# USharma002/CUDA-PathTracer

Measured on AMD Instinct MI355X. Metric: Msamples/s, higher is better.
Workload: dtype f32

## Files before the change

### cuda-pathtracer_amd/csrc/bounce.h

```cpp
#pragma once
#include "shading.h"

namespace ptmi {

struct BounceArgs {
    DeviceScene sc; TileMap tm; PathState st; FrameParams fp;
    const int* queue_in; int n_in;
    const int* count_in;
    int* queue_out; int* count_out;
    int segments;
    StatCounters* stats;
    int many_waves;
    int* done_count;
    int* next_count;
    int* host_count;
    int* cursor;
    unsigned int* cost; unsigned int* cost_max;
};

using BounceKernel = void (*)(BounceArgs);
#pragma GCC visibility push(hidden)
BounceKernel select_bounce_sync(const BounceArgs& a);
BounceKernel select_bounce_phased(const BounceArgs& a);
BounceKernel select_bounce_wide(const BounceArgs& a);
#pragma GCC visibility pop

inline bool is_guided(const BounceArgs& a) { return a.fp.sampling_mode != 0 && a.sc.cdfs != nullptr; }

#ifdef PTMI_TRACE_WAVES
#define PTMI_TR(...) __VA_ARGS__
#else
#define PTMI_TR(...)
#endif

template <bool LDS_GEOM>
__device__ __forceinline__ float4* stage_scene(const DeviceScene& sc, float4* lds, const float4*& nodes, const float4*& prims, const float4*& mats) {
    nodes = sc.nodes; prims = sc.prims; mats = sc.mats;
    if (LDS_GEOM) {
        const int n_node_vec = 2 * sc.n_nodes, n_prim_vec = sc.prim_stride * sc.n_prims, n_mat_vec = 3 * sc.n_prims;
        for (int i = threadIdx.x; i < n_node_vec; i += kBlock) lds[i] = sc.nodes[i];
        for (int i = threadIdx.x; i < n_prim_vec; i += kBlock) lds[n_node_vec + i] = sc.prims[i];
        for (int i = threadIdx.x; i < n_mat_vec; i += kBlock) lds[n_node_vec + n_prim_vec + i] = sc.mats[i];
        nodes = lds; prims = lds + n_node_vec; mats = lds + n_node_vec + n_prim_vec;
        lds += n_node_vec + n_prim_vec + n_mat_vec;
        __syncthreads();
    }
    return lds;
}

template <bool STATS, bool COMPACT = true>
__device__ __forceinline__ void finish_launch(const BounceArgs& a, bool alive, int slot, const LaneCounters& cn) {
    if (COMPACT) {
        const unsigned long long mask = __ballot(alive);
        const int lane = threadIdx.x & 63;
        int base = 0;
        if (lane == 0 && mask) base = atomicAdd(a.count_out, __popcll(mask));
        base = __shfl(base, 0);
        if (alive) a.queue_out[base + __popcll(mask & ((1ull << lane) - 1ull))] = slot;
    }
    if (STATS) {
        unsigned long long r = cn.rays, nv = cn.node_visits, pt = cn.prim_tests, h = cn.hits, tv = cn.top_visits;
        unsigned long long cc = cn.cert_chain, cf = cn.cert_fallback;
        for (int off = 32; off > 0; off >>= 1) {
            r += __shfl_down(r, off); nv += __shfl_down(nv, off); pt += __shfl_down(pt, off); h += __shfl_down(h, off); tv += __shfl_down(tv, off);
            cc += __shfl_down(cc, off); cf += __shfl_down(cf, off);
        }
        if ((threadIdx.x & 63) == 0) {
            atomicAdd(&a.stats->rays, r); atomicAdd(&a.stats->node_visits, nv);
            atomicAdd(&a.stats->prim_tests, pt); atomicAdd(&a.stats->hits, h);
            if (tv) atomicAdd(&a.stats->top_node_visits, tv);
            if (cc) atomicAdd(&a.stats->cert_chain, cc);
            if (cf) atomicAdd(&a.stats->cert_fallback, cf);
        }
    }
}

__device__ __forceinline__ void publish_count(const BounceArgs& a) {
    if (!a.host_count) return;
    if ((threadIdx.x & 63) == 0) {
        __threadfence();
        if (atomicAdd(a.done_count, 1) == (int)(gridDim.x * (kBlock / 64)) - 1) {
            const int c = atomicAdd(a.count_out, 0);
            atomicExch(a.next_count, 0); atomicExch(a.next_count + 1, 0);
            atomicExch(a.done_count, 0);
            __hip_atomic_store(a.host_count, c, __ATOMIC_RELEASE, __HIP_MEMORY_SCOPE_SYSTEM);
        }
    }
}

__device__ __forceinline__ bool end_visit(const BounceArgs& a, int n_in, bool more, int& slot, PathRegs& p, int& segs_left) {
    store_path(a.st, slot, p);
    if (a.cost) {
        const unsigned int c = a.cost[slot] + (unsigned int)(a.segments - segs_left);
        a.cost[slot] = c;
        if (!more) atomicMax(a.cost_max, c);
    }
    const int lane = threadIdx.x & 63;
    const unsigned long long ending = __ballot(1), surviving = __ballot(more);
    const int first = __ffsll((long long)ending) - 1;
    int out_base = 0, in_base = 0;
    if (lane == first) {
        if (surviving) out_base = atomicAdd(a.count_out, __popcll(surviving));
        if (a.cursor) in_base = atomicAdd(a.cursor, __popcll(ending));
    }
    out_base = __shfl(out_base, first); in_base = __shfl(in_base, first);
    if (more) a.queue_out[out_base + __popcll(surviving & ((1ull << lane) - 1ull))] = slot;
    const int entry = (int)(gridDim.x * kBlock) + in_base + __popcll(ending & ((1ull << lane) - 1ull));
    if (!(a.cursor && entry < n_in)) return false;
    slot = a.queue_in ? a.queue_in[entry] : entry;
    load_path(a.st, a.tm, slot, p);
    segs_left = a.segments;
    return true;
}

}
```

### cuda-pathtracer_amd/csrc/bounce_sync.hip

```cpp
#include "bounce.h"

namespace ptmi {

template <int MODE, bool LDS_GEOM, bool HAS_QUADS, bool STATS, bool GUIDED, bool BATCH>
__device__ __forceinline__ void bounce_body(const BounceArgs& a) {
    extern __shared__ float4 smem[];
    static_assert(MODE != TRAVERSAL_SWEEP || LDS_GEOM, "the sweep reads the scene through LDS broadcasts");
    const int n_in = a.count_in ? *a.count_in : a.n_in;
    if ((int)(blockIdx.x * kBlock) >= n_in) return;
    const int idx = blockIdx.x * kBlock + threadIdx.x;
    const bool active = idx < n_in;
    const float4 *nodes, *prims, *mats;
    float4* lds = stage_scene<LDS_GEOM>(a.sc, smem, nodes, prims, mats);
    int* stack = reinterpret_cast<int*>(lds) + threadIdx.x;
    if (GUIDED) fill_grid_solid_angles();

    const int slot = active ? (a.queue_in ? a.queue_in[idx] : idx) : 0;
    bool alive = active;
    PathRegs p = {};
    if (active) load_path(a.st, a.tm, slot, p);
    LaneCounters cn = {0, 0, 0, 0, 0, 0, 0};

    for (int seg = 0; seg < a.segments; seg++) {
        if (!__any(alive)) break;
        float t = 0.0f; int k = -1;
        if (STATS && alive) cn.rays++;
        const bool hit = scene_intersect<MODE, HAS_QUADS, STATS>(nodes, prims, a.sc.prim_stride, a.sc.n_nodes, stack, alive,
                                                               p.o, p.d, 1e-4f, FLT_MAX, t, k, cn);
        constexpr bool LEAN = MODE == TRAVERSAL_SWEEP && !STATS && !GUIDED;
        if (alive) alive = shade_step<STATS, GUIDED, false, BATCH, LEAN>(a.fp, a.tm, MatSource{mats, nullptr, nullptr}, a.sc.cdfs, p, hit, t, k, cn, slot);
    }

    if (active) store_path(a.st, slot, p);
    finish_launch<STATS>(a, alive, slot, cn);
}
template <int MODE, bool LDS_GEOM, bool HAS_QUADS, bool STATS, bool GUIDED, bool BATCH>
__global__ __launch_bounds__(kBlock, GUIDED ? 6 : (BATCH && MODE == TRAVERSAL_SWEEP ? 8 : 1)) __attribute__((amdgpu_num_sgpr(80))) void ptmi_bounce(BounceArgs a) {
    bounce_body<MODE, LDS_GEOM, HAS_QUADS, STATS, GUIDED, BATCH>(a);
    publish_count(a);
}

BounceKernel select_bounce_sync(const BounceArgs& a) {
    const auto pick = [&](auto mode, auto geom) {
        return with_bool(a.sc.has_quads, [&](auto quads) {
            return with_bool(a.stats != nullptr, [&](auto stats) {
                return with_bool(is_guided(a), [&](auto guided) {
                    return with_bool(a.fp.n_frames > 1, [&](auto batch) -> BounceKernel {
                        return ptmi_bounce<decltype(mode)::value, decltype(geom)::value, decltype(quads)::value, decltype(stats)::value,
                                           decltype(guided)::value, decltype(batch)::value>;
                    });
                });
            });
        });
    };
    switch (a.sc.traversal) {
        case TRAVERSAL_SWEEP: return pick(std::integral_constant<int, TRAVERSAL_SWEEP>{}, std::true_type{});
        case TRAVERSAL_LANE: return with_bool(a.sc.lds_resident, [&](auto geom) { return pick(std::integral_constant<int, TRAVERSAL_LANE>{}, geom); });
        default: return with_bool(a.sc.lds_resident, [&](auto geom) { return pick(std::integral_constant<int, TRAVERSAL_STACK>{}, geom); });
    }
}

}
```

### cuda-pathtracer_amd/csrc/debug_hooks.hip

```cpp
#include "light_sample.h"
#include "../../include/ptmi.h"

namespace ptmi {

template <int MODE, bool HAS_QUADS>
__global__ __launch_bounds__(kBlock) void ptmi_debug_intersect_k(DeviceScene sc, int n, const float* o, const float* d, float t_min,
                                                                 float t_max, int* hit, int* prim, float* t_out, float* p_out, float* n_out) {
    extern __shared__ float4 smem[];
    int* stack = reinterpret_cast<int*>(smem) + threadIdx.x;
    const int i = blockIdx.x * kBlock + threadIdx.x;
    const bool live = i < n;
    const int j = live ? i : 0;
    const f3 ro = mk3(o[3 * j], o[3 * j + 1], o[3 * j + 2]), rd = mk3(d[3 * j], d[3 * j + 1], d[3 * j + 2]);
    LaneCounters cn = {0, 0, 0, 0, 0, 0, 0};
    float t = 0.0f; int k = -1;
    const bool h = scene_intersect<MODE, HAS_QUADS, false>(sc.nodes, sc.prims, sc.prim_stride, sc.n_nodes, stack, live, ro, rd, t_min, t_max, t, k, cn);
    if (!live) return;
    hit[i] = h ? 1 : 0;
    prim[i] = h ? __float_as_int(sc.mats[3 * k].w) : -1;
    t_out[i] = h ? t : 0.0f;
    const f3 p = h ? ro + t * rd : mk3(0, 0, 0);
    const f3 nn = h ? xyz(sc.mats[3 * k]) : mk3(0, 0, 0);
    p_out[3 * i] = p.x; p_out[3 * i + 1] = p.y; p_out[3 * i + 2] = p.z;
    n_out[3 * i] = nn.x; n_out[3 * i + 1] = nn.y; n_out[3 * i + 2] = nn.z;
}

void launch_debug_intersect(const DeviceScene& sc, int n, const float* o, const float* d, float t_min, float t_max,
                            int* hit, int* prim, float* t, float* p, float* nrm, hipStream_t s) {
    if (n <= 0) return;
    const size_t lds = (size_t)sc.stack_entries * kBlock * sizeof(int);
    const dim3 grid((n + kBlock - 1) / kBlock), block(kBlock);
    const int walk = sc.traversal == TRAVERSAL_PHASED || sc.traversal == TRAVERSAL_PACKED || sc.traversal == TRAVERSAL_CERTIFIED ? TRAVERSAL_LANE : sc.traversal;
    const auto launch = [&](auto mode) {
        with_bool(sc.has_quads, [&](auto quads) {
            hipLaunchKernelGGL((ptmi_debug_intersect_k<decltype(mode)::value, decltype(quads)::value>), grid, block, lds, s, sc, n, o, d, t_min, t_max, hit, prim, t, p, nrm);
        });
    };
    if (walk == TRAVERSAL_SWEEP) launch(std::integral_constant<int, TRAVERSAL_SWEEP>{});
    else if (walk == TRAVERSAL_LANE) launch(std::integral_constant<int, TRAVERSAL_LANE>{});
    else launch(std::integral_constant<int, TRAVERSAL_STACK>{});
}

template <bool QUADS>
__global__ __launch_bounds__(kBlock) void ptmi_debug_intersect_wide_k(DeviceScene sc, int n, const float* o, const float* d, float t_min,
                                                                      float t_max, int* hit, int* prim, float* t_out,
                                                                      unsigned long long* counts ) {
    extern __shared__ float4 smem[];
    const int i = blockIdx.x * kBlock + threadIdx.x;
    if (i >= n) return;
    const f3 ro = mk3(o[3 * i], o[3 * i + 1], o[3 * i + 2]), rd = mk3(d[3 * i], d[3 * i + 1], d[3 * i + 2]);
    float closest_t = t_max;
    bool tie = false;
    WideCounts wc = {0, 0};
    const int slot_hit = wide_closest_hit<QUADS, true>(sc, reinterpret_cast<uint2*>(smem) + threadIdx.x, ro, rd, t_min, closest_t, tie, wc);
    hit[i] = slot_hit >= 0 ? 1 : 0;
    prim[i] = slot_hit >= 0 ? sc.wload_index[slot_hit] : -1;
    t_out[i] = slot_hit >= 0 ? closest_t : 0.0f;
    if (counts) { atomicAdd(&counts[0], (unsigned long long)wc.node_visits); atomicAdd(&counts[1], (unsigned long long)wc.prim_tests); }
}
void launch_debug_intersect_wide(const DeviceScene& sc, int n, const float* o, const float* d, float t_min, float t_max,
                                 int* hit, int* prim, float* t, unsigned long long* counts, hipStream_t s) {
    if (n <= 0) return;
    const size_t lds = (size_t)sc.w_depth * kBlock * sizeof(uint2);
    const dim3 grid((n + kBlock - 1) / kBlock), block(kBlock);
    with_bool(sc.has_quads, [&](auto quads) {
        hipLaunchKernelGGL(ptmi_debug_intersect_wide_k<decltype(quads)::value>, grid, block, lds, s, sc, n, o, d, t_min, t_max, hit, prim, t, counts);
    });
}

__global__ void ptmi_debug_rng_k(const uint32_t* __restrict__ jump, unsigned long long seed_base, int n_pixels,
                                 const int* pixels, int count, float* out) {
    const int i = blockIdx.x * blockDim.x + threadIdx.x;
    if (i >= n_pixels) return;
    const unsigned int pix = (unsigned int)pixels[i];
    const unsigned long long seed = seed_base + (unsigned long long)pix;
    const uint32_t s0 = ((uint32_t)seed) ^ 0xaad26b49u, s1 = (uint32_t)(seed >> 32) ^ 0xf7dcefddu;
    const uint32_t t0 = 1099087573u * s0, t1 = 2591861531u * s1;
    uint32_t v[5] = {123456789u + t0, 362436069u ^ t0, 521288629u + t1, 88675123u ^ t1, 5783321u + t0};
    for (int k = 0; k < 32; k++) {
        if (!((pix >> k) & 1u)) continue;
        uint32_t r[5] = {0, 0, 0, 0, 0};
        for (int w = 0; w < 5; w++)
            for (int b = 0; b < 32; b++)
                if ((v[w] >> b) & 1u) for (int c = 0; c < 5; c++) r[c] ^= jump[(k * 160 + w * 32 + b) * 5 + c];
        for (int w = 0; w < 5; w++) v[w] = r[w];
    }
    Rng rng = {v[0], v[1], v[2], v[3], v[4], 6615241u + t1 + t0};
    for (int c = 0; c < count; c++) out[(size_t)i * count + c] = rng_uniform(rng);
}

void launch_debug_rng(const uint32_t* d_jump, uint64_t seed_base, int n_pixels, const int* pixels, int count, float* out, hipStream_t s) {
    if (n_pixels <= 0) return;
    hipLaunchKernelGGL(ptmi_debug_rng_k, dim3((n_pixels + 63) / 64), dim3(64), 0, s, d_jump, (unsigned long long)seed_base,
                       n_pixels, pixels, count, out);
}

__global__ void ptmi_debug_rcp_k(unsigned int first, unsigned long long count, unsigned long long* out ) {
    const unsigned long long stride = (unsigned long long)gridDim.x * blockDim.x;
    unsigned long long bad = 0, first_bad = ~0ull;
    for (unsigned long long i = blockIdx.x * (unsigned long long)blockDim.x + threadIdx.x; i < count; i += stride) {
        const unsigned int bits = first + (unsigned int)i;
        const float a = __uint_as_float(bits);
        const float want = 1.0f / a, got = rcp_exact_normal(a);
        if (__float_as_uint(want) != __float_as_uint(got) && !(want != want && got != got)) { bad++; if (first_bad == ~0ull) first_bad = bits; }
    }
    if (bad) { atomicAdd(&out[0], bad); atomicMin(&out[1], first_bad); }
}
void launch_debug_rcp(unsigned int first, unsigned long long count, unsigned long long* d_out, hipStream_t s) {
    hipLaunchKernelGGL(ptmi_debug_rcp_k, dim3(4096), dim3(256), 0, s, first, count, d_out);
}

__global__ void ptmi_debug_sqrt_k(unsigned int first, unsigned long long count, unsigned long long* out ) {
    const unsigned long long stride = (unsigned long long)gridDim.x * blockDim.x;
    unsigned long long bad = 0, first_bad = ~0ull;
    for (unsigned long long i = blockIdx.x * (unsigned long long)blockDim.x + threadIdx.x; i < count; i += stride) {
// ... 271 lines not shown
```

### cuda-pathtracer_amd/csrc/kernels.hip

```cpp
#include "bounce.h"

namespace ptmi {

__global__ __launch_bounds__(kBlock) void ptmi_render_init(TileMap tm, PathState st, const uint32_t* __restrict__ jump,
                                                           unsigned long long seed_base) {
    __shared__ uint32_t M[160 * 5];
    const int n = tm.local_rows * tm.width;
    const int slot = blockIdx.x * kBlock + threadIdx.x;
    const bool live = slot < n;
    int x = 0, y = 0;
    const unsigned int pix = live ? (unsigned int)global_pixel(tm, slot, x, y) : 0u;
    const unsigned long long seed = seed_base + (unsigned long long)pix;
    const uint32_t s0 = ((uint32_t)seed) ^ 0xaad26b49u;
    const uint32_t s1 = (uint32_t)(seed >> 32) ^ 0xf7dcefddu;
    const uint32_t t0 = 1099087573u * s0;
    const uint32_t t1 = 2591861531u * s1;
    uint32_t v[5] = {123456789u + t0, 362436069u ^ t0, 521288629u + t1, 88675123u ^ t1, 5783321u + t0};
    const uint32_t d = 6615241u + t1 + t0;

    for (int k = 0; k < 32; k++) {
        const bool mine = live && ((pix >> k) & 1u);
        if (!__syncthreads_or(mine ? 1 : 0)) continue;
        for (int i = threadIdx.x; i < 160 * 5; i += kBlock) M[i] = jump[k * 160 * 5 + i];
        __syncthreads();
        if (mine) {
            uint32_t r[5] = {0u, 0u, 0u, 0u, 0u};
#pragma unroll
            for (int w = 0; w < 5; w++) {
                const uint32_t word = v[w];
                for (int b = 0; b < 32; b++) {
                    const uint32_t m = 0u - ((word >> b) & 1u);
                    const uint32_t* row = &M[(w * 32 + b) * 5];
                    r[0] ^= row[0] & m; r[1] ^= row[1] & m; r[2] ^= row[2] & m; r[3] ^= row[3] & m; r[4] ^= row[4] & m;
                }
            }
#pragma unroll
            for (int w = 0; w < 5; w++) v[w] = r[w];
        }
        __syncthreads();
    }
    if (!live) return;
    st.E[slot] = make_uint4(v[0], v[1], v[2], v[3]);
    st.F[slot] = make_uint2(v[4], d);
    st.A[slot] = make_float4(0, 0, 0, 1.0f);
    st.B[slot] = make_float4(0, 0, 1.0f, 1.0f);
    st.C[slot] = make_float4(0, 0, 0, 1.0f);
    st.D[slot] = make_float4(0, 0, 0, __uint_as_float(0u));
}

__global__ __launch_bounds__(kBlock) void ptmi_frame_begin(TileMap tm, PathState st, FrameParams fp) {
    const int n = tm.local_rows * tm.width;
    const int slot = blockIdx.x * kBlock + threadIdx.x;
    if (slot >= n) return;
    int x, y;
    global_pixel(tm, slot, x, y);
    const uint4 e = st.E[slot]; const uint2 f = st.F[slot];
    Rng rng = {e.x, e.y, e.z, e.w, f.x, f.y};
    f3 o, d;
    camera_ray(fp, tm, x, y, rng, o, d);
    st.A[slot] = make_float4(o.x, o.y, o.z, 1.0f);
    st.B[slot] = make_float4(d.x, d.y, d.z, 1.0f);
    st.C[slot] = make_float4(0.0f, 0.0f, 0.0f, 1.0f);
    st.D[slot] = make_float4(0.0f, 0.0f, 0.0f, __uint_as_float(0u));
    st.E[slot] = make_uint4(rng.v0, rng.v1, rng.v2, rng.v3);
    st.F[slot] = make_uint2(rng.v4, rng.d);
}

size_t bounce_lds_bytes_wide(const DeviceScene& sc) { return (size_t)sc.w_top * kWideNodeDwords * 4 + (size_t)sc.w_depth * kBlock * sizeof(uint2); }
size_t bounce_lds_bytes(const DeviceScene& sc) {
    if (sc.traversal == TRAVERSAL_WIDE || sc.traversal == TRAVERSAL_CERTIFIED) return bounce_lds_bytes_wide(sc);
    size_t b = 0;
    const bool geom = sc.lds_resident || sc.traversal == TRAVERSAL_SWEEP;
    if (geom) b += (size_t)(2 * sc.n_nodes + (sc.prim_stride + 3) * sc.n_prims) * sizeof(float4);
    if (sc.traversal == TRAVERSAL_STACK) b += (size_t)sc.stack_entries * kBlock * sizeof(int);
    return b;
}

static BounceKernel select_bounce_kernel(const BounceArgs& a, size_t* lds) {
    const DeviceScene& sc = a.sc;
    *lds = bounce_lds_bytes(sc);
    switch (sc.traversal) {
        case TRAVERSAL_PHASED: return select_bounce_phased(a);
        case TRAVERSAL_PACKED: *lds = (size_t)sc.n_top * 2 * sizeof(float4); return select_bounce_phased(a);
        case TRAVERSAL_WIDE:
        case TRAVERSAL_CERTIFIED: return select_bounce_wide(a);
        default: return select_bounce_sync(a);
    }
}

void launch_bounce(const DeviceScene& sc, const TileMap& tm, const PathState& st, const FrameParams& fp,
                   const int* queue_in, int n_in, const int* count_in, int* queue_out, int* count_out, int segments,
                   StatCounters* stats, bool many_waves, hipStream_t s, const CountPublish& pub, const LaunchSchedule& sched) {
    if (n_in <= 0) return;
    BounceArgs a{sc, tm, st, fp, queue_in, n_in, count_in, queue_out, count_out, segments, stats, many_waves ? 1 : 0,
                 pub.done_count, pub.next_count, pub.host_count, nullptr, nullptr, nullptr};
    dim3 grid((n_in + kBlock - 1) / kBlock);
    const bool wide = sc.traversal == TRAVERSAL_WIDE || sc.traversal == TRAVERSAL_CERTIFIED;
    if (wide && sched.max_waves > 0 && sched.cursor) {
        a.cursor = sched.cursor;
        grid.x = std::min<unsigned int>(grid.x, (unsigned int)(sched.max_waves + kBlock / 64 - 1) / (kBlock / 64));
    }
    if (wide) { a.cost = sched.cost; a.cost_max = sched.cost_max; }
    size_t lds = 0;
    const BounceKernel k = select_bounce_kernel(a, &lds);
    hipLaunchKernelGGL(k, grid, dim3(kBlock), lds, s, a);
}

int bounce_resident_waves(const DeviceScene& sc, const FrameParams& fp, bool stats, int n_cus) {
    BounceArgs a{sc, TileMap(), PathState(), fp, nullptr, 0, nullptr, nullptr, nullptr, 0, stats ? reinterpret_cast<StatCounters*>(1) : nullptr, 0,
                 nullptr, nullptr, nullptr, nullptr, nullptr, nullptr};
    size_t lds = 0;
    const BounceKernel k = select_bounce_kernel(a, &lds);
    int blocks = 0;
    if (hipOccupancyMaxActiveBlocksPerMultiprocessor(&blocks, k, kBlock, lds) != hipSuccess) blocks = 0;
    return blocks * (kBlock / 64) * n_cus;
}

__device__ __forceinline__ int cost_class(unsigned int c, unsigned int cmax, int shift) {
    const unsigned long long k = ((unsigned long long)min(c, cmax) << 8) / ((unsigned long long)cmax + 1ull);
    return (255 - (int)k) >> shift;
}
__global__ __launch_bounds__(kBlock) void ptmi_cost_histogram(const int* __restrict__ queue_in, int n, const unsigned int* __restrict__ cost,
                                                              const unsigned int* __restrict__ cost_max, int* __restrict__ hist, int shift) {
    __shared__ int h[256];
    h[threadIdx.x] = 0;
    __syncthreads();
    const unsigned int cmax = *cost_max;
    for (int i = blockIdx.x * kBlock + threadIdx.x; i < n; i += gridDim.x * kBlock)
        atomicAdd(&h[cost_class(cost[queue_in ? queue_in[i] : i], cmax, shift)], 1);
    __syncthreads();
    if (h[threadIdx.x]) atomicAdd(&hist[threadIdx.x], h[threadIdx.x]);
}
__global__ __launch_bounds__(kBlock) void ptmi_cost_offsets(int* __restrict__ hist) {
    __shared__ int h[256];
    h[threadIdx.x] = hist[threadIdx.x];
    __syncthreads();
    if (threadIdx.x == 0) { int acc = 0; for (int c = 0; c < 256; c++) { const int v = h[c]; h[c] = acc; acc += v; } }
    __syncthreads();
    hist[256 + threadIdx.x] = h[threadIdx.x];
}
__global__ __launch_bounds__(kBlock) void ptmi_cost_scatter(const int* __restrict__ queue_in, int n, const unsigned int* __restrict__ cost,
                                                            const unsigned int* __restrict__ cost_max, int* __restrict__ hist, int* __restrict__ queue, int shift) {
    __shared__ int h[256], base[256];
    __shared__ unsigned char cls[kBlock];
    h[threadIdx.x] = 0;
    const int i = blockIdx.x * kBlock + threadIdx.x;
    const int entry = i < n ? (queue_in ? queue_in[i] : i) : 0;
    const int c = i < n ? cost_class(cost[entry], *cost_max, shift) : 255;
    cls[threadIdx.x] = (unsigned char)c;
    __syncthreads();
    if (i < n) atomicAdd(&h[c], 1);
    int local = 0;
    for (int j = 0; j < (int)threadIdx.x; j++) local += cls[j] == c ? 1 : 0;
    __syncthreads();
    if (h[threadIdx.x]) base[threadIdx.x] = atomicAdd(&hist[256 + threadIdx.x], h[threadIdx.x]);
    __syncthreads();
// ... 131 lines not shown
```

### cuda-pathtracer_amd/csrc/traversal.h

```cpp
#pragma once
#include "pt_device.h"
#include "wide_walk.h"

namespace ptmi {

struct LaneCounters { unsigned int rays, node_visits, prim_tests, hits, top_visits, cert_chain, cert_fallback; };

__device__ __forceinline__ bool box_hit(const float4& n0, const float4& n1, f3 o, f3 inv, float t_min, float closest_t) {
    float t0x = (n0.x - o.x) * inv.x, t1x = (n1.x - o.x) * inv.x;
    if (inv.x < 0.0f) { const float tmp = t0x; t0x = t1x; t1x = tmp; }
    float t0y = (n0.y - o.y) * inv.y, t1y = (n1.y - o.y) * inv.y;
    if (inv.y < 0.0f) { const float tmp = t0y; t0y = t1y; t1y = tmp; }
    float t0z = (n0.z - o.z) * inv.z, t1z = (n1.z - o.z) * inv.z;
    if (inv.z < 0.0f) { const float tmp = t0z; t0z = t1z; t1z = tmp; }
    const float tmin_box = max3_raw(max_raw(t0x, t_min), t0y, t0z);
    const float tmax_box = min3_raw(min_raw(t1x, closest_t), t1y, t1z);
    return !(tmax_box < tmin_box);
}

__device__ __forceinline__ f3 ray_inv(f3 d, bool live) {
    float lo;
    asm("v_min3_f32 %0, |%1|, |%2|, |%3|" : "=v"(lo) : "v"(d.x), "v"(d.y), "v"(d.z));
    const float sum = fabsf(d.x) + fabsf(d.y) + fabsf(d.z);
    const bool in_range = (lo >= 0x1p-100f) & (sum <= 0x1p+100f);
    if (__any(live && !in_range)) return mk3(rcp_rn(d.x), rcp_rn(d.y), rcp_rn(d.z));
    return mk3(rcp_exact_normal(d.x), rcp_exact_normal(d.y), rcp_exact_normal(d.z));
}

template <bool HAS_QUADS>
__device__ __forceinline__ void leaf_prim(const float4* __restrict__ prims, int prim_stride, int k, f3 o, f3 d, float t_lo,
                                          float& closest_t, int& slot_hit) {
    const float4 p0 = prims[k * prim_stride], p1 = prims[k * prim_stride + 1], p2 = prims[k * prim_stride + 2];
    const float eps = 1e-8f, eps_up = __uint_as_float(__float_as_uint(1e-8f) + 1u);
    float t;
    if (HAS_QUADS && __float_as_int(p0.w) != 0) {
        const float4 p3 = prims[k * prim_stride + 3];
        const float t1 = mt_candidate(xyz(p0), xyz(p1), xyz(p2), o, d, eps_up, t_lo);
        const float c1 = min_raw(t1, closest_t);
        const float t2 = mt_candidate(xyz(p0), xyz(p2), xyz(p3), o, d, eps_up, t_lo);
        t = min_raw(t2, c1);
    } else {
        float tt = 0.0f;
        const bool acc = mt_accept(xyz(p0), xyz(p1), xyz(p2), o, d, eps, t_lo, closest_t, tt);
        closest_t = acc ? tt : closest_t;
        slot_hit = acc ? k : slot_hit;
        return;
    }
    const bool closer = t < closest_t;
    closest_t = min_raw(t, closest_t);
    slot_hit = closer ? k : slot_hit;
}

__device__ __forceinline__ void leaf_prim_packed(const float* __restrict__ gprims, int k, f3 o, f3 d, float t_lo, float& closest_t, int& slot_hit) {
    const f3p* r = reinterpret_cast<const f3p*>(gprims) + 3 * (size_t)k;
    const f3p v0 = r[0], e1 = r[1], e2 = r[2];
    float tt = 0.0f;
    const bool acc = mt_accept(mk3(v0.x, v0.y, v0.z), mk3(e1.x, e1.y, e1.z), mk3(e2.x, e2.y, e2.z), o, d, 1e-8f, t_lo, closest_t, tt);
    closest_t = acc ? tt : closest_t;
    slot_hit = acc ? k : slot_hit;
}

template <bool HAS_QUADS, bool STATS>
__device__ __forceinline__ bool intersect_stack(const float4* __restrict__ nodes, const float4* __restrict__ prims, int prim_stride,
                                                int* stack, bool live, f3 o, f3 d, float t_min, float t_max,
                                                float& t_hit, int& slot_hit, LaneCounters& cn) {
    float closest_t = t_max;
    slot_hit = -1;
    const f3 inv = ray_inv(d, live);
    const float t_lo = mt_t_lo(t_min);
    int sp = 0;
    int cur = live ? 0 : -1;
    while (true) {
        if (cur < 0) {
            if (sp == 0) break;
            cur = stack[(--sp) * kBlock];
        }
        const float4 n0 = nodes[2 * cur], n1 = nodes[2 * cur + 1];
        if (STATS) cn.node_visits++;
        const int here = cur;
        cur = -1;
        if (!box_hit(n0, n1, o, inv, t_min, closest_t)) continue;
        const int a = __float_as_int(n0.w), b = __float_as_int(n1.w);
        if (b < 0) {
            for (int i = 0; i < -b; i++) {
                if (STATS) cn.prim_tests++;
                leaf_prim<HAS_QUADS>(prims, prim_stride, a + i, o, d, t_lo, closest_t, slot_hit);
            }
        } else if (sp < 62) {
            stack[(sp++) * kBlock] = b;
            cur = here + 1;
        }
    }
    t_hit = closest_t;
    return slot_hit >= 0;
}

template <bool HAS_QUADS, bool STATS>
__device__ __forceinline__ bool intersect_lane(const float4* __restrict__ nodes, const float4* __restrict__ prims, int prim_stride,
                                               int n_nodes, bool live, f3 o, f3 d, float t_min, float t_max,
                                               float& t_hit, int& slot_hit, LaneCounters& cn) {
    float closest_t = t_max;
    slot_hit = -1;
    const f3 inv = ray_inv(d, live);
    const float t_lo = mt_t_lo(t_min);
    int cur = live ? 0 : n_nodes;
    while (cur < n_nodes) {
        const float4 n0 = nodes[2 * cur], n1 = nodes[2 * cur + 1];
        if (STATS) cn.node_visits++;
        const int a = __float_as_int(n0.w), b = __float_as_int(n1.w);
        const bool pass = box_hit(n0, n1, o, inv, t_min, closest_t);
        int next = cur + 1;
        if (!pass && b >= 0) next = a;
        if (pass && b < 0) {
            for (int i = 0; i < -b; i++) {
                if (STATS) cn.prim_tests++;
                leaf_prim<HAS_QUADS>(prims, prim_stride, a + i, o, d, t_lo, closest_t, slot_hit);
            }
        }
        cur = next;
    }
    t_hit = closest_t;
    return slot_hit >= 0;
}

template <bool HAS_QUADS>
__device__ __forceinline__ void leaf_prim_uniform(const float4* prims, int prim_stride, int k, f3 o, f3 d, float t_lo,
                                                  float& closest_t, int& slot_hit) {
    const float4 p0 = prims[k * prim_stride], p1 = prims[k * prim_stride + 1], p2 = prims[k * prim_stride + 2];
    const float eps = 1e-8f, eps_up = __uint_as_float(__float_as_uint(1e-8f) + 1u);
    float t;
    if (HAS_QUADS && __builtin_amdgcn_readfirstlane(__float_as_int(p0.w)) != 0) {
        const float4 p3 = prims[k * prim_stride + 3];
        const float t1 = mt_candidate(xyz(p0), xyz(p1), xyz(p2), o, d, eps_up, t_lo);
        const float c1 = min_raw(t1, closest_t);
        const float t2 = mt_candidate(xyz(p0), xyz(p2), xyz(p3), o, d, eps_up, t_lo);
        t = min_raw(t2, c1);
    } else {
        float tt = 0.0f;
        const bool acc = mt_accept(xyz(p0), xyz(p1), xyz(p2), o, d, eps, t_lo, closest_t, tt);
        closest_t = acc ? tt : closest_t;
        slot_hit = acc ? k : slot_hit;
        return;
    }
    const bool closer = t < closest_t;
    closest_t = min_raw(t, closest_t);
    slot_hit = closer ? k : slot_hit;
}

template <bool HAS_QUADS, bool STATS>
__device__ __forceinline__ bool intersect_sweep(const float4* nodes, const float4* prims, int prim_stride,
                                                int n_nodes, bool live, f3 o, f3 d, float t_min, float t_max,
                                                float& t_hit, int& slot_hit, LaneCounters& cn) {
    float closest_t = t_max;
    slot_hit = -1;
    const f3 inv = ray_inv(d, live);
    const float t_lo = mt_t_lo(t_min);
    int cur = live ? 0 : n_nodes;
    for (int n = 0; n < n_nodes; n++) {
        if (cur == n) {
            const int nu = __builtin_amdgcn_readfirstlane(n);
            const float4 n0 = nodes[2 * nu], n1 = nodes[2 * nu + 1];
            if (STATS) cn.node_visits++;
            const int a = __builtin_amdgcn_readfirstlane(__float_as_int(n0.w));
            const int b = __builtin_amdgcn_readfirstlane(__float_as_int(n1.w));
            const bool pass = box_hit(n0, n1, o, inv, t_min, closest_t);
            cur = n + 1;
            if (b < 0) {
                if (pass) {
                    for (int i = 0; i < -b; i++) {
                        if (STATS) cn.prim_tests++;
                        leaf_prim_uniform<HAS_QUADS>(prims, prim_stride, a + i, o, d, t_lo, closest_t, slot_hit);
                    }
                }
            } else if (!pass) cur = a;
        }
    }
    t_hit = closest_t;
    return slot_hit >= 0;
}

template <int MODE, bool HAS_QUADS, bool STATS>
__device__ __forceinline__ bool scene_intersect(const float4* __restrict__ nodes, const float4* __restrict__ prims, int prim_stride,
                                                int n_nodes, int* stack, bool live, f3 o, f3 d, float t_min, float t_max,
                                                float& t_hit, int& slot_hit, LaneCounters& cn) {
    if (MODE == TRAVERSAL_SWEEP) return intersect_sweep<HAS_QUADS, STATS>(nodes, prims, prim_stride, n_nodes, live, o, d, t_min, t_max, t_hit, slot_hit, cn);
    if (MODE == TRAVERSAL_LANE) return intersect_lane<HAS_QUADS, STATS>(nodes, prims, prim_stride, n_nodes, live, o, d, t_min, t_max, t_hit, slot_hit, cn);
    return intersect_stack<HAS_QUADS, STATS>(nodes, prims, prim_stride, stack, live, o, d, t_min, t_max, t_hit, slot_hit, cn);
}

template <bool QUADS>
__device__ __forceinline__ bool certified_closest_hit(const DeviceScene& sc, uint2* stack, f3 o, f3 d, float t_min, float& t_hit, int& ref_slot) {
    LaneCounters cn = {0, 0, 0, 0, 0, 0, 0};
    auto reference_walk = [&]() { return intersect_lane<QUADS, false>(sc.nodes, sc.prims, sc.prim_stride, sc.n_nodes, true, o, d, t_min, FLT_MAX, t_hit, ref_slot, cn); };
    if (!wide_origin_ok(sc, o)) return reference_walk();
    float closest_t = FLT_MAX;
    bool tie = false;
    WideCounts wc = {0, 0};
    const int slot_hit = wide_closest_hit<QUADS, false>(sc, stack, o, d, t_min, closest_t, tie, wc);
    if (slot_hit < 0) return false;
    if (tie) return reference_walk();
    const float4 lo = sc.wcert[kWideCertStride * (size_t)slot_hit], hi = sc.wcert[kWideCertStride * (size_t)slot_hit + 1];
    const f3 q = o + closest_t * d;
    const f3 rinv = mk3(rcp_rn(d.x), rcp_rn(d.y), rcp_rn(d.z));
    const bool proven = (CERT_LEAF_INSIDE(o, q, lo, hi) && CERT_SLOPES_OK(d, kCertSlope)) ||
                        cert_chain(sc, lo, o, d, closest_t, kCertSlope, [=](const float4& n0, const float4& n1) { return box_hit(n0, n1, o, rinv, t_min, closest_t); });
    if (!proven) return reference_walk();
    t_hit = closest_t;
    ref_slot = sc.wref_slot[slot_hit];
    return true;
}

template <int MODE, bool HAS_QUADS>
__device__ __forceinline__ bool first_hit(const DeviceScene& sc, float4* smem, bool live, f3 o, f3 d, float t_min, float& t, int& k, LaneCounters& cn) {
    bool hit;
    if constexpr (MODE == TRAVERSAL_CERTIFIED) hit = live && certified_closest_hit<HAS_QUADS>(sc, reinterpret_cast<uint2*>(smem) + threadIdx.x, o, d, t_min, t, k);
    else hit = scene_intersect<MODE, HAS_QUADS, false>(sc.nodes, sc.prims, sc.prim_stride, sc.n_nodes, reinterpret_cast<int*>(smem) + threadIdx.x, live, o, d, t_min, FLT_MAX, t, k, cn);
    return hit;
}

}
```

### cuda-pathtracer_amd/host/scene_state.cpp

```cpp
#include "application_state.h"

#include <algorithm>
#include <cfloat>
#include <cmath>
#include <cstring>

namespace ptmi {

void SceneState::cleanup() {
    if (d_nodes) (void)hipFree(d_nodes);
    if (d_prims) (void)hipFree(d_prims);
    if (d_mats) (void)hipFree(d_mats);
    if (d_precomputed_cdfs) (void)hipFree(d_precomputed_cdfs);
    if (d_radiosity) (void)hipFree(d_radiosity);
    if (d_emit_rec) (void)hipFree(d_emit_rec);
    if (d_emit_cdf) (void)hipFree(d_emit_cdf);
    if (d_pdf_area) (void)hipFree(d_pdf_area);
    if (d_surfaces) (void)hipFree(d_surfaces);
    d_surfaces = nullptr; n_mirror = n_glass = 0;
    for (int& c : surface_counts) c = 0;
    d_emit_rec = d_pdf_area = nullptr; d_emit_cdf = nullptr; d_emitters = EmitterTable();
    h_emit_prim.clear(); h_emit_cdf.clear(); h_emit_normal.clear(); h_pdf_area.clear(); h_emit_total = 0.0f;
    freePacked();
    freeFast();
// ... 463 lines not shown
            }
            nd = (float2*)hipMallocSafe((size_t)n * sizeof(float2), "d_surfaces");
            const hipError_t e = hipMemcpy(nd, slot.data(), (size_t)n * sizeof(float2), hipMemcpyHostToDevice);
            if (e != hipSuccess) { (void)hipFree(nd); PTMI_HIP(e); }
        }
    }
    if (d_surfaces) (void)hipFree(d_surfaces);
    d_surfaces = nd; n_mirror = mirrors; n_glass = glasses;
    const bool table = nd != nullptr;
    surface_counts[0] = table ? n - mirrors - glasses - roughs : 0;
    surface_counts[1] = mirrors; surface_counts[2] = glasses; surface_counts[3] = roughs;
}


void SceneState::precomputeCDFsDevice(const void* d_src, int src_kind, hipStream_t stream) {
    if (!d_nodes) throw ArgError("precomputeCDFs: no scene loaded");
    if (d_precomputed_cdfs) { (void)hipFree(d_precomputed_cdfs); d_precomputed_cdfs = nullptr; }
    h_precomputed_cdfs.clear();
    d_scene.cdfs = nullptr;
    const int n = (int)h_primitives.size();
    d_precomputed_cdfs = (float*)hipMallocSafe((size_t)n * kCdfDwords * sizeof(float), "d_precomputed_cdfs");
    launch_cdf_records(n, d_src, src_kind, d_precomputed_cdfs, stream);
    PTMI_HIP(hipGetLastError());
    PTMI_HIP(hipStreamSynchronize(stream));
    d_scene.cdfs = d_precomputed_cdfs;
}

const std::vector<float>& SceneState::precomputedCdfsHost() {
    if (h_precomputed_cdfs.empty() && d_precomputed_cdfs) {
        h_precomputed_cdfs.resize(h_primitives.size() * (size_t)kCdfDwords);
        PTMI_HIP(hipMemcpy(h_precomputed_cdfs.data(), d_precomputed_cdfs, h_precomputed_cdfs.size() * sizeof(float), hipMemcpyDeviceToHost));
    }
    return h_precomputed_cdfs;
}

void SceneState::precomputeCDFs(const float* rgb) {
    if (!d_nodes) throw ArgError("precomputeCDFs: no scene loaded");
    if (d_precomputed_cdfs) { (void)hipFree(d_precomputed_cdfs); d_precomputed_cdfs = nullptr; }
    h_precomputed_cdfs.clear();
    d_scene.cdfs = nullptr;
    h_filtered_formfactor.clear(); h_filtered_radiosity.clear();
    if (!rgb) { h_radiosity_grids.clear(); return; }
    const size_t cells = h_primitives.size() * (size_t)kGridSize;
    if (rgb != h_radiosity_grids.data()) h_radiosity_grids.assign(rgb, rgb + cells * 3);
    struct Tmp { void* p = nullptr; ~Tmp() { if (p) (void)hipFree(p); } } d_rgb;
    d_rgb.p = hipMallocSafe(cells * 3 * sizeof(float), "d_radiosity_grids_rgb");
    PTMI_HIP(hipMemcpy(d_rgb.p, rgb, cells * 3 * sizeof(float), hipMemcpyHostToDevice));
    precomputeCDFsDevice(d_rgb.p, 1, nullptr);
}

void SceneState::precomputeCDFsFromFiltered(bool use_bilateral, float sigma_spatial, float sigma_range, hipStream_t stream) {
    if (!d_nodes) throw ArgError("precomputeCDFsFromFiltered: no scene loaded");
    if (h_radiosity_grids.empty()) throw ArgError("precomputeCDFsFromFiltered: the scene has no radiosity grids");
    const int n = (int)h_primitives.size();
    const size_t cells = (size_t)n * kGridSize;
    struct Tmp { void* p = nullptr; ~Tmp() { if (p) (void)hipFree(p); } } rgb, cnt, off, orad;
    rgb.p = hipMallocSafe(cells * 3 * sizeof(float), "d_filter_rgb");
    off.p = hipMallocSafe(cells * sizeof(float), "d_filtered_formfactor");
    orad.p = hipMallocSafe(cells * sizeof(float), "d_filtered_radiosity");
    PTMI_HIP(hipMemcpy(rgb.p, h_radiosity_grids.data(), cells * 3 * sizeof(float), hipMemcpyHostToDevice));
    if (!h_count_grids.empty()) {
        cnt.p = hipMallocSafe(cells * sizeof(float), "d_filter_counts");
        PTMI_HIP(hipMemcpy(cnt.p, h_count_grids.data(), cells * sizeof(float), hipMemcpyHostToDevice));
    }
    launch_filter_pdfs(n, (const float*)rgb.p, (const float*)cnt.p, (float*)off.p, (float*)orad.p, use_bilateral, sigma_spatial, sigma_range, stream);
    PTMI_HIP(hipGetLastError());
    PTMI_HIP(hipStreamSynchronize(stream));
    h_filtered_formfactor.resize(cells); h_filtered_radiosity.resize(cells);
    PTMI_HIP(hipMemcpy(h_filtered_formfactor.data(), off.p, cells * sizeof(float), hipMemcpyDeviceToHost));
    PTMI_HIP(hipMemcpy(h_filtered_radiosity.data(), orad.p, cells * sizeof(float), hipMemcpyDeviceToHost));
    precomputeCDFsDevice(orad.p, 2, stream);
}

void SceneState::chooseTraversal() {
    if (!d_nodes) return;
    if (bvh_depth > 62) d_scene.traversal = TRAVERSAL_STACK;
    else if ((int)h_primitives.size() <= sweep_max_prims) d_scene.traversal = TRAVERSAL_SWEEP;
    else d_scene.traversal = certified_default && d_scene.certified_ready() ? TRAVERSAL_CERTIFIED : (d_scene.gnodes ? TRAVERSAL_PACKED : TRAVERSAL_PHASED);
    if (force_traversal >= 0 && !(force_traversal != TRAVERSAL_STACK && bvh_depth > 62)) d_scene.traversal = force_traversal;
    if (d_scene.traversal == TRAVERSAL_SWEEP && !d_scene.lds_resident) d_scene.traversal = TRAVERSAL_LANE;
    if (d_scene.traversal == TRAVERSAL_PACKED && !d_scene.gnodes) d_scene.traversal = TRAVERSAL_PHASED;
    if (d_scene.traversal == TRAVERSAL_CERTIFIED && !d_scene.certified_ready())
        d_scene.traversal = (int)h_primitives.size() <= sweep_max_prims && d_scene.lds_resident ? TRAVERSAL_SWEEP : (d_scene.gnodes ? TRAVERSAL_PACKED : TRAVERSAL_PHASED);
}

}
```

### cuda-pathtracer_amd/python/ptmi_buildinfo.py

```python
import hashlib
import os

_HERE = os.path.dirname(os.path.abspath(__file__))
PKG = os.path.dirname(_HERE)
ROOT = os.path.dirname(PKG)

def _csrc(*names):
    return [os.path.join(PKG, "csrc", n) for n in names]


_SHARED_SOURCES = _csrc("pt_device.h", "pt_vec.h", "device_scene.h", "wide_bvh.h", "wide_walk.h", "prim_sample.h") + [
    os.path.join(ROOT, "include", "ptmi_math.h"), os.path.join(PKG, "Makefile")]
KERNEL_SOURCES = _csrc("kernels.hip", "bounce_sync.hip", "bounce_phased.hip", "bounce_wide.hip", "first_hit.hip", "debug_hooks.hip",
                       "traversal.h", "shading.h", "shade_lean.h", "bounce.h") + _SHARED_SOURCES + [
    os.path.join(PKG, "host", "render_run.cpp"), os.path.join(PKG, "host", "launch_rule.h"),
    os.path.join(PKG, "host", "wide_bvh.cpp"),
]
SOLVER_SOURCES = _csrc("radiosity.hip", "form_factors.hip", "anyhit.h") + _SHARED_SOURCES + [os.path.join(PKG, "host", "radiosity_state.cpp")]


def _sha(paths):
    h = hashlib.sha256()
    for p in paths:
        h.update(os.path.basename(p).encode() + b"\0")
        with open(p, "rb") as f:
            h.update(f.read())
    return h.hexdigest()


def lib_sha256():
    p = os.environ.get("PTMI_LIB") or os.path.join(PKG, "libptmi.so")
    if not os.path.exists(p):
        return None
    with open(p, "rb") as f:
        return hashlib.sha256(f.read()).hexdigest()


def kernel_src_sha256():
    return _sha(KERNEL_SOURCES)


def solver_src_sha256():
    return _sha(SOLVER_SOURCES)


def stamps():
    return {"lib_sha256": lib_sha256(), "kernel_src_sha256": kernel_src_sha256(), "solver_src_sha256": solver_src_sha256()}


def profile_is_current(profile, solver=False):
    if profile.get("lib_sha256") and profile.get("lib_sha256") == lib_sha256():
        return True, "lib"
    if solver:
        if profile.get("solver_src_sha256") and profile.get("solver_src_sha256") == solver_src_sha256():
            return True, "solver_sources"
        return False, None
    if profile.get("kernel_src_sha256") and profile.get("kernel_src_sha256") == kernel_src_sha256():
        return True, "kernel_sources"
    return False, None
```

Baseline: 7663.

## Rewrite sweep traversal over LDS byte-address records with pre-resolved skip pointers

When staging the scene into LDS for the sweep traversal, node skip indices are rewritten into LDS byte addresses and each primitive's record gets its slot id embedded. The sweep loop then walks raw LDS addresses, unrolls leaf tests by four, and uses a voted early-out Moller-Trumbore update plus a single select for the next node in the triangle-only case. This removes index-to-address arithmetic and scalar readfirstlane work in the hot loop. Quad scenes without stats also get a higher occupancy hint. It adds asm register pinning and a stride invariant check, and changes the debug kernel to stage the scene the same way.

```diff
diff --git a/cuda-pathtracer_amd/csrc/bounce.h b/cuda-pathtracer_amd/csrc/bounce.h
--- a/cuda-pathtracer_amd/csrc/bounce.h
+++ b/cuda-pathtracer_amd/csrc/bounce.h
@@ -1,5 +1,6 @@
 #pragma once
 #include "shading.h"
+#include "sweep_records.h"
 
 namespace ptmi {
 
@@ -33,13 +34,20 @@
 #define PTMI_TR(...)
 #endif
 
-template <bool LDS_GEOM>
+template <bool LDS_GEOM, bool SWEEP_RECORDS = false>
 __device__ __forceinline__ float4* stage_scene(const DeviceScene& sc, float4* lds, const float4*& nodes, const float4*& prims, const float4*& mats) {
+    static_assert(LDS_GEOM || !SWEEP_RECORDS, "the sweep's records exist in LDS only");
     nodes = sc.nodes; prims = sc.prims; mats = sc.mats;
     if (LDS_GEOM) {
         const int n_node_vec = 2 * sc.n_nodes, n_prim_vec = sc.prim_stride * sc.n_prims, n_mat_vec = 3 * sc.n_prims;
-        for (int i = threadIdx.x; i < n_node_vec; i += kBlock) lds[i] = sc.nodes[i];
-        for (int i = threadIdx.x; i < n_prim_vec; i += kBlock) lds[n_node_vec + i] = sc.prims[i];
+        if (SWEEP_RECORDS) {
+            ptmi_sweep_prepare(reinterpret_cast<const ptmi_vec_bits*>(sc.nodes), sc.n_nodes, reinterpret_cast<const ptmi_vec_bits*>(sc.prims),
+                               sc.prim_stride, sc.n_prims, reinterpret_cast<ptmi_vec_bits*>(lds), reinterpret_cast<ptmi_vec_bits*>(lds + n_node_vec),
+                               lds_address(lds), (int)threadIdx.x, kBlock);
+        } else {
+            for (int i = threadIdx.x; i < n_node_vec; i += kBlock) lds[i] = sc.nodes[i];
+            for (int i = threadIdx.x; i < n_prim_vec; i += kBlock) lds[n_node_vec + i] = sc.prims[i];
+        }
         for (int i = threadIdx.x; i < n_mat_vec; i += kBlock) lds[n_node_vec + n_prim_vec + i] = sc.mats[i];
         nodes = lds; prims = lds + n_node_vec; mats = lds + n_node_vec + n_prim_vec;
         lds += n_node_vec + n_prim_vec + n_mat_vec;
diff --git a/cuda-pathtracer_amd/csrc/bounce_sync.hip b/cuda-pathtracer_amd/csrc/bounce_sync.hip
--- a/cuda-pathtracer_amd/csrc/bounce_sync.hip
+++ b/cuda-pathtracer_amd/csrc/bounce_sync.hip
@@ -11,7 +11,7 @@
     const int idx = blockIdx.x * kBlock + threadIdx.x;
     const bool active = idx < n_in;
     const float4 *nodes, *prims, *mats;
-    float4* lds = stage_scene<LDS_GEOM>(a.sc, smem, nodes, prims, mats);
+    float4* lds = stage_scene<LDS_GEOM, MODE == TRAVERSAL_SWEEP>(a.sc, smem, nodes, prims, mats);
     int* stack = reinterpret_cast<int*>(lds) + threadIdx.x;
     if (GUIDED) fill_grid_solid_angles();
 
@@ -35,7 +35,7 @@
     finish_launch<STATS>(a, alive, slot, cn);
 }
 template <int MODE, bool LDS_GEOM, bool HAS_QUADS, bool STATS, bool GUIDED, bool BATCH>
-__global__ __launch_bounds__(kBlock, GUIDED ? 6 : (BATCH && MODE == TRAVERSAL_SWEEP ? 8 : 1)) __attribute__((amdgpu_num_sgpr(80))) void ptmi_bounce(BounceArgs a) {
+__global__ __launch_bounds__(kBlock, GUIDED ? 6 : ((BATCH || (HAS_QUADS && !STATS)) && MODE == TRAVERSAL_SWEEP ? 8 : 1)) __attribute__((amdgpu_num_sgpr(80))) void ptmi_bounce(BounceArgs a) {
     bounce_body<MODE, LDS_GEOM, HAS_QUADS, STATS, GUIDED, BATCH>(a);
     publish_count(a);
 }
diff --git a/cuda-pathtracer_amd/csrc/debug_hooks.hip b/cuda-pathtracer_amd/csrc/debug_hooks.hip
--- a/cuda-pathtracer_amd/csrc/debug_hooks.hip
+++ b/cuda-pathtracer_amd/csrc/debug_hooks.hip
@@ -1,3 +1,4 @@
+#include "bounce.h"
 #include "light_sample.h"
 #include "../../include/ptmi.h"
 
@@ -8,13 +9,15 @@
                                                                  float t_max, int* hit, int* prim, float* t_out, float* p_out, float* n_out) {
     extern __shared__ float4 smem[];
     int* stack = reinterpret_cast<int*>(smem) + threadIdx.x;
+    const float4 *nodes, *prims, *mats;
+    stage_scene<MODE == TRAVERSAL_SWEEP, MODE == TRAVERSAL_SWEEP>(sc, smem, nodes, prims, mats);
     const int i = blockIdx.x * kBlock + threadIdx.x;
     const bool live = i < n;
     const int j = live ? i : 0;
     const f3 ro = mk3(o[3 * j], o[3 * j + 1], o[3 * j + 2]), rd = mk3(d[3 * j], d[3 * j + 1], d[3 * j + 2]);
     LaneCounters cn = {0, 0, 0, 0, 0, 0, 0};
     float t = 0.0f; int k = -1;
-    const bool h = scene_intersect<MODE, HAS_QUADS, false>(sc.nodes, sc.prims, sc.prim_stride, sc.n_nodes, stack, live, ro, rd, t_min, t_max, t, k, cn);
+    const bool h = scene_intersect<MODE, HAS_QUADS, false>(nodes, prims, sc.prim_stride, sc.n_nodes, stack, live, ro, rd, t_min, t_max, t, k, cn);
     if (!live) return;
     hit[i] = h ? 1 : 0;
     prim[i] = h ? __float_as_int(sc.mats[3 * k].w) : -1;
@@ -28,9 +31,9 @@
 void launch_debug_intersect(const DeviceScene& sc, int n, const float* o, const float* d, float t_min, float t_max,
                             int* hit, int* prim, float* t, float* p, float* nrm, hipStream_t s) {
     if (n <= 0) return;
-    const size_t lds = (size_t)sc.stack_entries * kBlock * sizeof(int);
     const dim3 grid((n + kBlock - 1) / kBlock), block(kBlock);
-    const int walk = sc.traversal == TRAVERSAL_PHASED || sc.traversal == TRAVERSAL_PACKED || sc.traversal == TRAVERSAL_CERTIFIED ? TRAVERSAL_LANE : sc.traversal;
+    const size_t lds = sc.traversal == TRAVERSAL_SWEEP ? bounce_lds_bytes(sc) : (size_t)sc.stack_entries * kBlock * sizeof(int);
+    const int walk =sc.traversal == TRAVERSAL_PHASED || sc.traversal == TRAVERSAL_PACKED || sc.traversal == TRAVERSAL_CERTIFIED ? TRAVERSAL_LANE : sc.traversal;
     const auto launch = [&](auto mode) {
         with_bool(sc.has_quads, [&](auto quads) {
             hipLaunchKernelGGL((ptmi_debug_intersect_k<decltype(mode)::value, decltype(quads)::value>), grid, block, lds, s, sc, n, o, d, t_min, t_max, hit, prim, t, p, nrm);
diff --git a/cuda-pathtracer_amd/csrc/kernels.hip b/cuda-pathtracer_amd/csrc/kernels.hip
--- a/cuda-pathtracer_amd/csrc/kernels.hip
+++ b/cuda-pathtracer_amd/csrc/kernels.hip
@@ -71,7 +71,7 @@
     if (sc.traversal == TRAVERSAL_WIDE || sc.traversal == TRAVERSAL_CERTIFIED) return bounce_lds_bytes_wide(sc);
     size_t b = 0;
     const bool geom = sc.lds_resident || sc.traversal == TRAVERSAL_SWEEP;
-    if (geom) b += (size_t)(2 * sc.n_nodes + (sc.prim_stride + 3) * sc.n_prims) * sizeof(float4);
+    if (geom) b += ptmi_scene_lds_vecs(sc.n_nodes, sc.prim_stride, sc.n_prims) * sizeof(float4);
     if (sc.traversal == TRAVERSAL_STACK) b += (size_t)sc.stack_entries * kBlock * sizeof(int);
     return b;
 }
diff --git a/cuda-pathtracer_amd/csrc/sweep_records.h b/cuda-pathtracer_amd/csrc/sweep_records.h
--- /dev/null
+++ b/cuda-pathtracer_amd/csrc/sweep_records.h
@@ -0,0 +1,38 @@
+#ifndef PTMI_SWEEP_RECORDS_H
+#define PTMI_SWEEP_RECORDS_H
+
+#include <stddef.h>
+
+#include "../../include/ptmi_math.h"
+
+#define PTMI_SWEEP_VEC_BYTES 16
+#define PTMI_SWEEP_NODE_BYTES (2 * PTMI_SWEEP_VEC_BYTES)
+
+typedef struct __attribute__((aligned(16))) { uint32_t x, y, z, w; } ptmi_vec_bits;
+
+PTMI_HD size_t ptmi_scene_lds_vecs(int n_nodes, int prim_stride, int n_prims) {
+    return 2 * (size_t)n_nodes + ((size_t)prim_stride + 3) * (size_t)n_prims;
+}
+
+PTMI_HD void ptmi_sweep_prepare(const ptmi_vec_bits* nodes, int n_nodes, const ptmi_vec_bits* prims, int prim_stride, int n_prims,
+                                ptmi_vec_bits* out_nodes, ptmi_vec_bits* out_prims, uint32_t nodes_at, int first, int step) {
+    int i, k, c;
+    for (i = first; i < n_nodes; i += step) {
+        ptmi_vec_bits n0 = nodes[2 * i];
+        const ptmi_vec_bits n1 = nodes[2 * i + 1];
+        if ((int32_t)n1.w >= 0) n0.w = nodes_at + n0.w * (uint32_t)PTMI_SWEEP_NODE_BYTES;
+        out_nodes[2 * i] = n0;
+        out_nodes[2 * i + 1] = n1;
+    }
+    for (k = first; k < n_prims; k += step) {
+        const ptmi_vec_bits* r = prims + (size_t)prim_stride * k;
+        ptmi_vec_bits* o = out_prims + (size_t)prim_stride * k;
+        ptmi_vec_bits e1 = r[1];
+        e1.w = (uint32_t)k;
+        o[0] = r[0];
+        o[1] = e1;
+        for (c = 2; c < prim_stride; c++) o[c] = r[c];
+    }
+}
+
+#endif
diff --git a/cuda-pathtracer_amd/csrc/traversal.h b/cuda-pathtracer_amd/csrc/traversal.h
--- a/cuda-pathtracer_amd/csrc/traversal.h
+++ b/cuda-pathtracer_amd/csrc/traversal.h
@@ -1,5 +1,6 @@
 #pragma once
 #include "pt_device.h"
+#include "sweep_records.h"
 #include "wide_walk.h"
 
 namespace ptmi {
@@ -123,56 +124,135 @@
     return slot_hit >= 0;
 }
 
+enum : int { SWEEP_VOTED_UPDATE = 1, SWEEP_PINNED = 2, SWEEP_LEAF_BASE = 4, SWEEP_ONE_SELECT = 8 };
+constexpr int kSweepLeafUnroll = 4;
+
 template <bool HAS_QUADS>
-__device__ __forceinline__ void leaf_prim_uniform(const float4* prims, int prim_stride, int k, f3 o, f3 d, float t_lo,
-                                                  float& closest_t, int& slot_hit) {
-    const float4 p0 = prims[k * prim_stride], p1 = prims[k * prim_stride + 1], p2 = prims[k * prim_stride + 2];
-    const float eps = 1e-8f, eps_up = __uint_as_float(__float_as_uint(1e-8f) + 1u);
-    float t;
+constexpr int sweep_form() { return HAS_QUADS ? 0 : (SWEEP_ONE_SELECT | SWEEP_VOTED_UPDATE | SWEEP_PINNED | SWEEP_LEAF_BASE); }
+
+__device__ __forceinline__ void mt_accept_update(f3 v0, f3 edge1, f3 edge2, f3 o, f3 d, float eps_for_a, float t_lo, int slot,
+                                                 float& closest_t, int& slot_hit) {
+    const f3 h = cross(d, edge2);
+    const float a = dot(edge1, h);
+    const float f = rcp_exact_normal(a);
+    const f3 s = o - v0;
+    const float u = f * dot(s, h);
+    const float m1 = min3_raw(fabsf(a) - eps_for_a, u, 1.0f - u);
+    if (!__any(m1 >= 0.0f)) return;
+    const f3 q = cross(s, edge1);
+    const float v = f * dot(d, q);
+    const float t = f * dot(edge2, q);
+    float m = min3_raw(m1, v, 1.0f - (u + v));
+    m = min_raw(m, t - t_lo);
+    const bool acc = (m >= 0.0f) & (t < closest_t);
+    closest_t = acc ? t : closest_t;
+    slot_hit = acc ? slot : slot_hit;
+}
+__device__ __forceinline__ unsigned int lds_address(const void* p) {
+#if defined(__HIP_DEVICE_COMPILE__)
+    return (unsigned int)(uintptr_t)(const __attribute__((address_space(3))) void*)p;
+#else
+    return 0u;
+#endif
+}
+__device__ __forceinline__ float4 lds_vec(unsigned int address, int i) {
+#if defined(__HIP_DEVICE_COMPILE__)
+    typedef float vec4 __attribute__((ext_vector_type(4)));
+    const vec4 v = reinterpret_cast<const __attribute__((address_space(3))) vec4*>(address)[i];
+    return make_float4(v.x, v.y, v.z, v.w);
+#else
+    return make_float4(0.0f, 0.0f, 0.0f, 0.0f);
+#endif
+}
+
+template <bool HAS_QUADS, int FORM>
+__device__ __forceinline__ void leaf_prim_sweep(unsigned int rec, int at, f3 o, f3 d, float eps, float eps_up, float t_lo,
+                                                float& closest_t, int& slot_hit) {
+    const float4 p0 = lds_vec(rec, at), p1 = lds_vec(rec, at + 1), p2 = lds_vec(rec, at + 2);
+    const int slot = __float_as_int(p1.w);
+    constexpr bool VOTED = (FORM & SWEEP_VOTED_UPDATE) != 0;
     if (HAS_QUADS && __builtin_amdgcn_readfirstlane(__float_as_int(p0.w)) != 0) {
-        const float4 p3 = prims[k * prim_stride + 3];
-        const float t1 = mt_candidate(xyz(p0), xyz(p1), xyz(p2), o, d, eps_up, t_lo);
-        const float c1 = min_raw(t1, closest_t);
-        const float t2 = mt_candidate(xyz(p0), xyz(p2), xyz(p3), o, d, eps_up, t_lo);
-        t = min_raw(t2, c1);
+        const float4 p3 = lds_vec(rec, at + 3);
+        if (VOTED) {
+            mt_accept_update(xyz(p0), xyz(p1), xyz(p2), o, d, eps_up, t_lo, slot, closest_t, slot_hit);
+            mt_accept_update(xyz(p0), xyz(p2), xyz(p3), o, d, eps_up, t_lo, slot, closest_t, slot_hit);
+        } else {
+            const float t1 = mt_candidate(xyz(p0), xyz(p1), xyz(p2), o, d, eps_up, t_lo);
+            const float c1 = min_raw(t1, closest_t);
+            const float t2 = mt_candidate(xyz(p0), xyz(p2), xyz(p3), o, d, eps_up, t_lo);
+            const float t = min_raw(t2, c1);
+            const bool closer = t < closest_t;
+            closest_t = min_raw(t, closest_t);
+            slot_hit = closer ? slot : slot_hit;
+        }
+    } else if (VOTED) {
+        mt_accept_update(xyz(p0), xyz(p1), xyz(p2), o, d, eps, t_lo, slot, closest_t, slot_hit);
     } else {
         float tt = 0.0f;
         const bool acc = mt_accept(xyz(p0), xyz(p1), xyz(p2), o, d, eps, t_lo, closest_t, tt);
         closest_t = acc ? tt : closest_t;
-        slot_hit = acc ? k : slot_hit;
-        return;
-    }
-    const bool closer = t < closest_t;
-    closest_t = min_raw(t, closest_t);
-    slot_hit = closer ? k : slot_hit;
-}
-
-template <bool HAS_QUADS, bool STATS>
-__device__ __forceinline__ bool intersect_sweep(const float4* nodes, const float4* prims, int prim_stride,
-                                                int n_nodes, bool live, f3 o, f3 d, float t_min, float t_max,
-                                                float& t_hit, int& slot_hit, LaneCounters& cn) {
+        slot_hit = acc ? slot : slot_hit;
+    }
+}
+
+template <bool HAS_QUADS, bool STATS, int FORM>
+__device__ __forceinline__ bool intersect_sweep(const float4* nodes, const float4* prims, int n_nodes, bool live, f3 o, f3 d,
+                                                float t_min, float t_max, float& t_hit, int& slot_hit, LaneCounters& cn) {
+    constexpr int kPrimVecs = HAS_QUADS ? 4 : 3;
+    constexpr unsigned int kPrimBytes = kPrimVecs * PTMI_SWEEP_VEC_BYTES;
     float closest_t = t_max;
     slot_hit = -1;
     const f3 inv = ray_inv(d, live);
-    const float t_lo = mt_t_lo(t_min);
-    int cur = live ? 0 : n_nodes;
-    for (int n = 0; n < n_nodes; n++) {
-        if (cur == n) {
-            const int nu = __builtin_amdgcn_readfirstlane(n);
-            const float4 n0 = nodes[2 * nu], n1 = nodes[2 * nu + 1];
+    float t_lo = mt_t_lo(t_min), eps = 1e-8f, eps_up = __uint_as_float(__float_as_uint(1e-8f) + 1u);
+    if (FORM & SWEEP_PINNED) {
+        asm("" : "+v"(t_lo));
+        asm("" : "+v"(eps));
+        if (HAS_QUADS) asm("" : "+v"(eps_up));
+    }
+    const unsigned int first = lds_address(nodes), end = first + (unsigned int)n_nodes * PTMI_SWEEP_NODE_BYTES;
+    const unsigned int prims_at = lds_address(prims);
+    unsigned int cur = live ? first : end;
+    for (unsigned int at = first; at < end; at += PTMI_SWEEP_NODE_BYTES) {
+        if (cur == at) {
+            unsigned int here = cur;
+            asm("" : "+v"(here));
+            const float4 n0 = lds_vec(here, 0), n1 = lds_vec(here, 1);
             if (STATS) cn.node_visits++;
-            const int a = __builtin_amdgcn_readfirstlane(__float_as_int(n0.w));
             const int b = __builtin_amdgcn_readfirstlane(__float_as_int(n1.w));
             const bool pass = box_hit(n0, n1, o, inv, t_min, closest_t);
-            cur = n + 1;
-            if (b < 0) {
-                if (pass) {
+            const unsigned int next = here + PTMI_SWEEP_NODE_BYTES, skip = __float_as_uint(n0.w);
+            const auto leaf_pass = [&]() {
+                const unsigned int leaf = prims_at + (unsigned int)__builtin_amdgcn_readfirstlane(__float_as_int(n0.w)) * kPrimBytes;
+                if constexpr ((FORM & SWEEP_LEAF_BASE) != 0) {
+                    unsigned int rec = leaf;
+                    asm("" : "+v"(rec));
+                    const auto test = [&](int i) {
+                        if (STATS) cn.prim_tests++;
+                        leaf_prim_sweep<HAS_QUADS, FORM>(rec, i * kPrimVecs, o, d, eps, eps_up, t_lo, closest_t, slot_hit);
+                    };
+                    static_assert(kSweepLeafUnroll == 4, "the four calls below");
+                    for (int left = -b; left > 0; left -= kSweepLeafUnroll, rec += kSweepLeafUnroll * kPrimBytes) {
+                        test(0);
+                        if (left > 1) test(1);
+                        if (left > 2) test(2);
+                        if (left > 3) test(3);
+                    }
+                } else {
                     for (int i = 0; i < -b; i++) {
                         if (STATS) cn.prim_tests++;
-                        leaf_prim_uniform<HAS_QUADS>(prims, prim_stride, a + i, o, d, t_lo, closest_t, slot_hit);
+                        leaf_prim_sweep<HAS_QUADS, FORM>(leaf + i * kPrimBytes, 0, o, d, eps, eps_up, t_lo, closest_t, slot_hit);
                     }
                 }
-            } else if (!pass) cur = a;
+            };
+            if constexpr ((FORM & SWEEP_ONE_SELECT) != 0) {
+                cur = ((b >= 0) & !pass) ? skip : next;
+                if (b < 0 && pass) leaf_pass();
+            } else if (b < 0) {
+                cur = next;
+                if (pass) leaf_pass();
+            } else {
+                cur = pass ? next : skip;
+            }
         }
     }
     t_hit = closest_t;
@@ -183,7 +263,7 @@
 __device__ __forceinline__ bool scene_intersect(const float4* __restrict__ nodes, const float4* __restrict__ prims, int prim_stride,
                                                 int n_nodes, int* stack, bool live, f3 o, f3 d, float t_min, float t_max,
                                                 float& t_hit, int& slot_hit, LaneCounters& cn) {
-    if (MODE == TRAVERSAL_SWEEP) return intersect_sweep<HAS_QUADS, STATS>(nodes, prims, prim_stride, n_nodes, live, o, d, t_min, t_max, t_hit, slot_hit, cn);
+    if (MODE == TRAVERSAL_SWEEP) return intersect_sweep<HAS_QUADS, STATS, sweep_form<HAS_QUADS>()>(nodes, prims, n_nodes, live, o, d, t_min, t_max, t_hit, slot_hit, cn);
     if (MODE == TRAVERSAL_LANE) return intersect_lane<HAS_QUADS, STATS>(nodes, prims, prim_stride, n_nodes, live, o, d, t_min, t_max, t_hit, slot_hit, cn);
     return intersect_stack<HAS_QUADS, STATS>(nodes, prims, prim_stride, stack, live, o, d, t_min, t_max, t_hit, slot_hit, cn);
 }
diff --git a/cuda-pathtracer_amd/host/scene_state.cpp b/cuda-pathtracer_amd/host/scene_state.cpp
--- a/cuda-pathtracer_amd/host/scene_state.cpp
+++ b/cuda-pathtracer_amd/host/scene_state.cpp
@@ -569,6 +569,8 @@
     if (d_scene.traversal == TRAVERSAL_PACKED && !d_scene.gnodes) d_scene.traversal = TRAVERSAL_PHASED;
     if (d_scene.traversal == TRAVERSAL_CERTIFIED && !d_scene.certified_ready())
         d_scene.traversal = (int)h_primitives.size() <= sweep_max_prims && d_scene.lds_resident ? TRAVERSAL_SWEEP : (d_scene.gnodes ? TRAVERSAL_PACKED : TRAVERSAL_PHASED);
-}
-
-}
+    if (d_scene.traversal == TRAVERSAL_SWEEP && d_scene.prim_stride != (d_scene.has_quads ? 4 : 3))
+        throw ArgError("internal: the sweep reads 3 float4 per primitive without quads and 4 with");
+}
+
+}
diff --git a/cuda-pathtracer_amd/python/ptmi_buildinfo.py b/cuda-pathtracer_amd/python/ptmi_buildinfo.py
--- a/cuda-pathtracer_amd/python/ptmi_buildinfo.py
+++ b/cuda-pathtracer_amd/python/ptmi_buildinfo.py
@@ -12,7 +12,7 @@
 _SHARED_SOURCES = _csrc("pt_device.h", "pt_vec.h", "device_scene.h", "wide_bvh.h", "wide_walk.h", "prim_sample.h") + [
     os.path.join(ROOT, "include", "ptmi_math.h"), os.path.join(PKG, "Makefile")]
 KERNEL_SOURCES = _csrc("kernels.hip", "bounce_sync.hip", "bounce_phased.hip", "bounce_wide.hip", "first_hit.hip", "debug_hooks.hip",
-                       "traversal.h", "shading.h", "shade_lean.h", "bounce.h") + _SHARED_SOURCES + [
+                       "traversal.h", "sweep_records.h", "shading.h", "shade_lean.h", "bounce.h") + _SHARED_SOURCES + [
     os.path.join(PKG, "host", "render_run.cpp"), os.path.join(PKG, "host", "launch_rule.h"),
     os.path.join(PKG, "host", "wide_bvh.cpp"),
 ]
```

Measured after the change: 8046, median of 6. 5.0% higher.
